# zju3dv/NeuralRecon-W

Hardware: AMD Instinct MI355X
Metric: ray-samples/sec (train step) at 1024 rays x 128 samples (higher is better)
Workload: dtype f16; 1 GPU; brandenburg_gate config (BASELINE.json configs[1]): 1024 rays/GPU x (64 coarse + 64 fine) samples, SDF 8x256 + colour 4x256 + bg NeRF 8x256, 4 outside samples, up_sample_steps 2, render+loss+backward+allreduce+clip+Adam; rays_per_gpu=1024, samples_per_ray=128, global_rays=1024, parallelism=dp1, world_size=1, submission=eager, streams=2, skipped_steps=0

## Files before the change

include/neuconw_hip.h:

```cpp
#ifndef NEUCONW_HIP_H
#define NEUCONW_HIP_H
#include <stdint.h>

#ifdef __cplusplus
extern "C" {
#endif

#define NCW_PREC_F32 0
#define NCW_PREC_BF16 1
#define NCW_PREC_F16 2
#define NCW_MAX_LAYERS 12
#define NCW_MAX_SEGS 4

#define NCW_E_BADARG (-1)
#define NCW_E_UNSUPPORTED (-2)

int ncw_abi_version(void);
const char* ncw_source_hash(void);
int ncw_device_info(char* buf, int buflen);

typedef struct NcwSeg {
    int32_t col0;
    int32_t ncols;
    int32_t dcol0;
// ... 136 lines not shown
    const void* w_p[8]; const void* wt_p[8]; const float* b_p[8];
    const void* w_alpha; const void* wt_alpha; const float* b_alpha;
    const void* w_feat; const void* wt_feat; const float* b_feat;
    const void* w_a[4]; const void* wt_a[4]; const float* b_a[4];
    const void* w_rgb; const void* wt_rgb; const float* b_rgb;
    int32_t D;
    int32_t skip;
    int32_t rbn, rbh, n_head, n_a;
    const void* w_p_lo[8]; const void* w_alpha_lo; const void* w_feat_lo; const void* w_a_lo[4]; const void* w_rgb_lo;
} NcwNerfNet;

typedef struct NcwNerfStash {
    void* gp;
    void* aux1;
    void* h[9];
    void* featn;
    void* e[4];
    void* zp[8];
    void* zalpha;
    void* zfeat;
    void* ze[4];
    void* zrgb;
    const float* aux_bias;
} NcwNerfStash;

int ncw_nerf_fwd(const NcwNerfNet* net, int prec, const NcwPoints* pts, const float* x4, int64_t n, const float* a,
                 float* density, float* rgb, const NcwNerfStash* stash, void* stream);
int ncw_nerf_bwd(const NcwNerfNet* net, int prec, const NcwPoints* pts, int64_t n, const float* d_density,
                 const float* d_rgb, float* d_a, float* d_a_rows, const NcwNerfStash* stash, void* stream);
int ncw_nerf_refine(const NcwNerfNet* net, int prec, const NcwPoints* pts, int64_t n, const float* aux_bias, float* density,
                    float* rgb, void* stream);
int ncw_batch_assemble(const float* all_rays, int ncols, const float* all_rgbs, const int64_t* idx, int64_t n_rows,
                       int64_t B, int with_semantics, float* rays, int64_t* ts, int64_t* label, float* rgbs,
                       const int* mask_ids, int n_ids, uint8_t* keep, void* stream);
int ncw_aux_ray_bias(const float* w, int ldw, int col0, int n_out, const float* rays_d, const float* a, int n_a, int64_t R,
                     float* out, int ldo, void* stream);
int ncw_ray_prologue(const float* rays, int ncols, int64_t R, const float* origin_host, float radius, float* rays_o,
                     float* rays_d, float* near, float* far, float* depth_gt, float* depth_weight, void* stream);
int ncw_inv_s_fwd(const float* variance, float* inv_s, float* s_val, void* stream);
int ncw_inv_s_bwd(const float* d_inv_s_rays, int64_t R, const float* inv_s, float* d_variance, void* stream);
int ncw_loss_fwd(const float* color, const float* rgbs, int64_t R, const float* gradient_error, const float* mask_error,
                 int64_t n_mask, const float* sfm, int64_t n_sfm, float coef, float igr_w, float mask_w, float depth_w,
                 float* loss, void* stream);
int ncw_loss_bwd(const float* d_loss, const float* color, const float* rgbs, int64_t R, int64_t n_mask, int64_t n_sfm,
                 float coef, float igr_w, float mask_w, float depth_w, float* d_color, float* d_gradient_error,
                 float* d_mask_error, float* d_sfm, void* stream);
// ... 325 lines not shown
```

neuralrecon-w_amd/csrc/ncw_mlp.h:

```cpp
#pragma once
#include "../../include/neuconw_hip.h"
#include "ncw_common.h"

template <class P>
struct Fast { static constexpr bool v = (P::id == NCW_PREC_BF16); };

NCW_DEV void ncw_lds_barrier() {
    asm volatile("s_waitcnt lgkmcnt(0)" ::: "memory");
    __builtin_amdgcn_s_barrier();
    asm volatile("" ::: "memory");
}

NCW_DEV float grid_linspace(float start, float end, int steps, int i) {
    if (steps == 1) return start;
    const float step = (end - start) / (float)(steps - 1);
    return (i < steps / 2) ? start + step * (float)i : end - step * (float)(steps - 1 - i);
}

NCW_DEV int64_t points_count(const NcwPoints& s, int64_t n) {
    if (s.mode != 4) return n;
    const int64_t c = (int64_t)s.count[0];
    return c < n ? c : n;
}
NCW_DEV int64_t point_slot(const NcwPoints& s, int64_t p) { return s.mode == 4 ? (int64_t)s.idx[p] : p; }
// ... 106 lines not shown
NCW_DEV void relu_epilogue(Act<P, RB>& act, CVec<RB>& acc, typename P::selem* st, size_t tile, int lane) {
#pragma unroll
    for (int rb = 0; rb < RB; ++rb) {
        f32x16 yv;
#pragma unroll
        for (int r = 0; r < 16; ++r) yv[r] = ncw_relu(acc.v[rb][r]);
        if (st) stash_store_block(st, tile, RB, rb, yv, lane);
        to_act_block<RB>(act, rb, yv);
    }
}

template <class P, int RB>
NCW_DEV void relu_backward(Act<P, RB>& za, const CVec<RB>& u, const typename P::selem* st_y, typename P::selem* st_z,
                           size_t tile, int lane) {
#pragma unroll
    for (int rb = 0; rb < RB; ++rb) {
        f32x16 y, z;
        stash_load_block(y, st_y, tile, RB, rb, lane);
#pragma unroll
        for (int r = 0; r < 16; ++r) z[r] = y[r] > 0.f ? u.v[rb][r] : 0.f;
        stash_store_block(st_z, tile, RB, rb, z, lane);
        to_act_block<RB>(za, rb, z);
    }
}

template <class P, int RB, int NX = 0>
struct SoftplusB {
    static constexpr int RB_IN = RB + NX;
    typedef typename P::selem SE;
    const CVec<RB>& z;
    SE* st_h;
    SE* st_s;
    size_t tile;
    int lane;
    const Act<P, (NX > 0 ? NX : 1)>* extra;
    Act<P, RB> act;
    NCW_DEV SoftplusB(const CVec<RB>& z_, SE* h, SE* s, size_t t, int l, const Act<P, (NX > 0 ? NX : 1)>* x = nullptr)
        : z(z_), st_h(h), st_s(s), tile(t), lane(l), extra(x) {}
    NCW_DEV void prepare(int rb) {
        if (rb >= RB) return;
        f32x16 yv, sv;
#pragma unroll
        for (int r = 0; r < 16; ++r) {
            float y, sg;
            softplus100<Fast<P>::v>(z.v[rb][r], y, sg);
            yv[r] = y;
// ... 173 lines not shown
```

neuralrecon-w_amd/csrc/ncw_sdf8.hip:

```cpp
#include "ncw_mlp.h"

namespace {

constexpr int SB_WAVES = 8, SB_TILES = 4;

NCW_DEV void load_sprime_block_bf16(f32x16& sv, const ncw_h16* __restrict__ st_h, size_t tile, int RB, int rb, int lane) {
    stash_load_block(sv, st_h, tile, RB, rb, lane);
#pragma unroll
    for (int r = 0; r < 16; ++r) sv[r] = 1.f - __builtin_amdgcn_exp2f(sv[r] * -144.26950408889634f);
}
constexpr int SB_ACT = SB_TILES * 16 * 1024;
constexpr int SB_GAM = SB_TILES * 3 * 1024;

typedef __attribute__((address_space(3))) bf16x8 sb_lfrag;

template <int NU>
NCW_DEV void sb_load_slice(bf16x8* a, const void* w, int rb_stride, int ob, int u0, int lane) {
#pragma unroll
    for (int q = 0; q < NU; ++q) a[q] = ncw_ld_frag<bf16x8>(w, (size_t)(u0 + q) * rb_stride + ob, lane);
}

constexpr int SB_RD = 4;

template <int NU, bool TWO, int NPF = 0>
// ... 230 lines not shown
        int comp;
        const float dv = freq_feature_deriv<3, 6, true>(xs, f0 + 4 * h, comp);
        const float c = gg[r] * dv;
        nx += comp == 0 ? c : 0.f;
        ny += comp == 1 ? c : 0.f;
        nz += comp == 2 ? c : 0.f;
    }
    nx = half_pair_sum(nx); ny = half_pair_sum(ny); nz = half_pair_sum(nz);
    typedef __attribute__((address_space(3))) float lfloat;
    lfloat* part = (lfloat*)gbuf;
    if (jb == 1 && lane < 32) {
        part[(jt * 32 + lane) * 3 + 0] = nx; part[(jt * 32 + lane) * 3 + 1] = ny; part[(jt * 32 + lane) * 3 + 2] = nz;
    }
    ncw_lds_barrier();
    if (jb == 0 && lane < 32 && valid) {
        grad[p * 3 + 0] = nx + part[(jt * 32 + lane) * 3 + 0];
        grad[p * 3 + 1] = ny + part[(jt * 32 + lane) * 3 + 1];
        grad[p * 3 + 2] = nz + part[(jt * 32 + lane) * 3 + 2];
    }
}


constexpr int SB_X = SB_TILES * 6 * 1024;

NCW_DEV void inverted_sphere8(const float (&x)[3], float (&p4)[4]) {
    float r2;
    {
#pragma clang fp contract(off)
        const float s1 = x[1] * x[1], s2 = x[2] * x[2];
        r2 = __builtin_fmaf(x[0], x[0], s1) + s2;
    }
    float r = sqrtf(r2);
    r = fminf(fmaxf(r, 1.0f), 1e10f);
    p4[0] = x[0] / r; p4[1] = x[1] / r; p4[2] = x[2] / r; p4[3] = 1.0f / r;
}

template <bool TRAIN>
__global__ __launch_bounds__(64 * SB_WAVES) void nerf_fwdB_kernel(NcwNerfNet net, NcwPoints src, const float* __restrict__ x4,
                                                                 int64_t n, const float* __restrict__ a,
                                                                 float* __restrict__ density, float* __restrict__ rgb,
                                                                 NcwNerfStash st) {
    typedef ncw_h16 SE;
    __shared__ __attribute__((aligned(16))) char lds[2 * SB_ACT + SB_X + SB_TILES * 32 * 4];
    sb_lfrag* const abuf0 = (sb_lfrag*)(ncw_lchar*)lds;
    sb_lfrag* const abuf1 = abuf0 + SB_ACT / 16;
    sb_lfrag* const xbuf = abuf0 + 2 * SB_ACT / 16;
    typedef __attribute__((address_space(3))) int sb_lint;
    sb_lint* const rbuf = (sb_lint*)(xbuf + SB_X / 16);
    const int lane = ncw_lane();
    const int wave = __builtin_amdgcn_readfirstlane((int)(threadIdx.x >> 6));
    const int64_t tile0 = (int64_t)blockIdx.x * SB_TILES;
    const int D = net.D;
    n = points_count(src, n);
    if (tile0 * 32 >= n) return;
    int64_t pp = 0;
    bool pvalid = false;
    if (wave < SB_TILES) {
        int64_t p = (tile0 + wave) * 32 + (lane & 31), ray;
        pvalid = p < n;
        if (!pvalid) p = n - 1;
// ... 28 lines not shown
        load_bias(b1, bp + ob * 32, lane);
        return b1.v[0];
    };
    auto relu16 = [](const f32x16& v) {
        f32x16 y;
#pragma unroll
        for (int r = 0; r < 16; ++r) y[r] = ncw_relu(v[r]);
        return y;
    };
    f32x16 bnext;
    {
        bf16x8 w0[6];
        const f32x16 bias = bias_of(net.b_p[0], wave);
        sb_load_slice<6>(w0, net.w_p[0], 8, wave, 0, lane);
        bnext = bias_of(D > 1 ? net.b_p[1] : net.b_feat, wave);
        sb_load_slice<16>(wa, D > 1 ? net.w_p[1] : net.w_feat, 8, wave, 0, lane);
        ncw_lds_barrier();
#pragma unroll
        for (int t = 0; t < SB_TILES; ++t) {
            f32x16 acc = bias;
            sb_mma<6, false>(acc, acc, w0, xbuf + t * 6 * 64 + lane, nullptr);
            const f32x16 y = relu16(acc);
            if (TRAIN) stash_store_block((SE*)st.h[1], (size_t)(tile0 + t), 8, wave, y, lane);
            sb_store_units(abuf0, t, wave, y, lane);
        }
    }
    int cur = 0;
    for (int i = 1; i < D; ++i) {
        const bool skip = (i == net.skip + 1);
        const void* wnext = i + 1 < D ? net.w_p[i + 1] : net.w_feat;
        const f32x16 bias = bnext;
        if (skip) sb_load_slice<6>(wx, net.w_p[i], 8, wave, 16, lane);
        bnext = bias_of(i + 1 < D ? net.b_p[i + 1] : net.b_feat, wave);
        ncw_lds_barrier();
        const sb_lfrag* in = cur ? abuf1 : abuf0;
        sb_lfrag* out = cur ? abuf0 : abuf1;
#pragma unroll
        for (int tp = 0; tp < SB_TILES; tp += 2) {
            f32x16 acc0 = bias, acc1 = bias;
            const sb_lfrag *in0 = in + tp * 16 * 64 + lane, *in1 = in0 + 16 * 64;
            if (tp == SB_TILES - 2) sb_mma<16, true, 16>(acc0, acc1, wa, in0, in1, wnext, 8, wave, lane);
            else sb_mma<16, true>(acc0, acc1, wa, in0, in1);
            if (skip) sb_mma<6, true>(acc0, acc1, wx, xbuf + tp * 6 * 64 + lane, xbuf + (tp + 1) * 6 * 64 + lane);
#pragma unroll
            for (int j = 0; j < 2; ++j) {
                const f32x16 y = relu16(j ? acc1 : acc0);
                if (TRAIN) stash_store_block((SE*)st.h[i + 1], (size_t)(tile0 + tp + j), 8, wave, y, lane);
                sb_store_units(out, tp + j, wave, y, lane);
            }
        }
        cur ^= 1;
    }
    const int hb = wave & 3, hp = wave >> 2;
    const int ta = 2 * hp, tb = 2 * hp + 1;
    {
        const f32x16 bias = bnext;
        ncw_lds_barrier();
        const sb_lfrag* in = cur ? abuf1 : abuf0;
        sb_lfrag* out = cur ? abuf0 : abuf1;
        if (wave < SB_TILES) {
            if (TRAIN || st.aux_bias == nullptr) {
                CVec<3> aux1;
                if (TRAIN) {
                    stash_load<3>(aux1, (const SE*)st.aux1, (size_t)(tile0 + wave), lane);
                } else {
                    const int64_t ray = rbuf[wave * 32 + (lane & 31)];
                    const float dir[3] = {src.rays_d[ray * 3 + 0], src.rays_d[ray * 3 + 1], src.rays_d[ray * 3 + 2]};
                    build_aux1<true>(aux1, dir, a + ray * net.n_a, net.n_a, lane);
                }
                Act<PrecBF16, 3> aux1a;
// ... 6 lines not shown
            sb_load_slice<16>(w1, net.w_alpha, 1, 0, 0, lane);
            CVec<1> o;
            load_bias(o, net.b_alpha, lane);
            sb_mma<16, false>(o.v[0], o.v[0], w1, in + wave * 16 * 64 + lane, nullptr);
            if (pvalid && lane < 32) density[pp] = o.v[0][0];
        }
        sb_load_slice<6>(wx, net.w_a[0], 4, hb, 16, lane);
        bnext = bias_of(net.b_a[0], hb);
#pragma unroll
        for (int tp = 0; tp < SB_TILES; tp += 2) {
            f32x16 acc0 = bias, acc1 = bias;
            const sb_lfrag *in0 = in + tp * 16 * 64 + lane, *in1 = in0 + 16 * 64;
            if (tp == SB_TILES - 2) sb_mma<16, true, 16>(acc0, acc1, wa, in0, in1, net.w_a[0], 4, hb, lane);
            else sb_mma<16, true>(acc0, acc1, wa, in0, in1);
            if (TRAIN) {
                stash_store_block((SE*)st.featn, (size_t)(tile0 + tp), 8, wave, acc0, lane);
                stash_store_block((SE*)st.featn, (size_t)(tile0 + tp + 1), 8, wave, acc1, lane);
            }
            sb_store_units(out, tp, wave, acc0, lane);
            sb_store_units(out, tp + 1, wave, acc1, lane);
        }
        cur ^= 1;
    }
    for (int i = 0; i < net.n_head; ++i) {
        const bool more = i + 1 < net.n_head;
        const f32x16 bias = bnext;
        if (more) bnext = bias_of(net.b_a[i + 1], hb);
        f32x16 rb0, rb1;
        const bool ray_rows = (i == 0 && st.aux_bias != nullptr);
        if (ray_rows) {
            auto ray_row = [&](int t) {
                const f32x4* ab = reinterpret_cast<const f32x4*>(st.aux_bias + (size_t)rbuf[t * 32 + (lane & 31)] * 128) + 8 * hb + (lane >> 5);
                f32x16 v;
#pragma unroll
                for (int g = 0; g < 4; ++g) {
                    const f32x4 q = ab[2 * g];
#pragma unroll
                    for (int c = 0; c < 4; ++c) v[4 * g + c] = q[c];
                }
                return v;
            };
            rb0 = ray_row(ta);
            rb1 = ray_row(tb);
        }
        ncw_lds_barrier();
        const sb_lfrag* in = cur ? abuf1 : abuf0;
        sb_lfrag* out = cur ? abuf0 : abuf1;
        const sb_lfrag *in0 = in + ta * 16 * 64 + lane, *in1 = in + tb * 16 * 64 + lane;
        const void* wnext = net.w_a[more ? i + 1 : i];
        f32x16 acc0 = bias, acc1 = bias;
        if (i == 0) {
            sb_mma<16, true, 8>(acc0, acc1, wa, in0, in1, wnext, 4, hb, lane);
            if (ray_rows) {
#pragma unroll
                for (int r = 0; r < 16; ++r) { acc0[r] += rb0[r]; acc1[r] += rb1[r]; }
            } else {
                sb_mma<6, true>(acc0, acc1, wx, xbuf + ta * 6 * 64 + lane, xbuf + tb * 6 * 64 + lane);
            }
        } else {
            sb_mma<8, true, 8>(acc0, acc1, wa, in0, in1, wnext, 4, hb, lane);
        }
        const f32x16 y0 = relu16(acc0), y1 = relu16(acc1);
        if (TRAIN) {
            stash_store_block((SE*)st.e[i], (size_t)(tile0 + ta), 4, hb, y0, lane);
            stash_store_block((SE*)st.e[i], (size_t)(tile0 + tb), 4, hb, y1, lane);
        }
        sb_store_units(out, ta, hb, y0, lane);
        sb_store_units(out, tb, hb, y1, lane);
        cur ^= 1;
    }
    ncw_lds_barrier();
    if (wave < SB_TILES) {
        const sb_lfrag* in = cur ? abuf1 : abuf0;
        bf16x8 w1[8];
        sb_load_slice<8>(w1, net.w_rgb, 1, 0, 0, lane);
        CVec<1> o;
        load_bias(o, net.b_rgb, lane);
        sb_mma<8, false>(o.v[0], o.v[0], w1, in + wave * 16 * 64 + lane, nullptr);
        if (pvalid && lane < 32) {
            rgb[pp * 3 + 0] = o.v[0][0];
            rgb[pp * 3 + 1] = o.v[0][1];
            rgb[pp * 3 + 2] = o.v[0][2];
        }
    }
}


typedef ncw_h16 sb_h4 __attribute__((ext_vector_type(4)));
struct SbMask { sb_h4 g[4]; };
NCW_DEV SbMask sb_mask_load(const ncw_h16* __restrict__ st_y, size_t tile, int RB, int rb, int lane) {
    const sb_h4* p = reinterpret_cast<const sb_h4*>(st_y) + ((tile * RB + rb) * 4) * 64 + lane;
    SbMask m;
#pragma unroll
    for (int g = 0; g < 4; ++g) m.g[g] = NCW_STASH_LD(p[g * 64]);
    return m;
}
NCW_DEV f32x16 sb_relu_bwd(const f32x16& u, const SbMask& m) {
    f32x16 z;
#pragma unroll
    for (int r = 0; r < 16; ++r) z[r] = (float)m.g[r >> 2][r & 3] > 0.f ? u[r] : 0.f;
    return z;
}

NCW_DEV void sb_accumulate_d_a(int rb, const f32x16& q, float* __restrict__ d_a, int64_t ray, int n_a, bool valid, int lane) {
    const int h = lane >> 5;
    const int64_t r0 = __shfl(ray, 0, 64);
    const bool uniform = __all((ray == r0) ? 1 : 0);
#pragma unroll
    for (int r = 0; r < 16; ++r) {
        const int f = 32 * rb + ncw_feat_of(r, 0) + 4 * h;
        const int j = f - 27;
        float v = valid ? q[r] : 0.f;
        if (uniform) {
#pragma unroll
            for (int o = 1; o < 32; o <<= 1) v += __shfl_xor(v, o, 64);
            if ((lane & 31) == 0 && j >= 0 && j < n_a) atomicAdd(d_a + ray * n_a + j, v);
        } else {
            if (valid && j >= 0 && j < n_a) atomicAdd(d_a + ray * n_a + j, v);
        }
    }
}

__global__ __launch_bounds__(64 * SB_WAVES) void nerf_bwdB_kernel(NcwNerfNet net, NcwPoints src, int64_t n,
                                                                 const float* __restrict__ d_density,
                                                                 const float* __restrict__ d_rgb, float* __restrict__ d_a,
                                                                 NcwNerfStash st) {
    typedef ncw_h16 SE;
    __shared__ __attribute__((aligned(16))) char lds[2 * SB_ACT + SB_X];
    sb_lfrag* const abuf0 = (sb_lfrag*)(ncw_lchar*)lds;
    sb_lfrag* const abuf1 = abuf0 + SB_ACT / 16;
    sb_lfrag* const xbuf = abuf0 + 2 * SB_ACT / 16;
    const int lane = ncw_lane();
    const int wave = __builtin_amdgcn_readfirstlane((int)(threadIdx.x >> 6));
    const int64_t tile0 = (int64_t)blockIdx.x * SB_TILES;
    const int D = net.D, NH = net.n_head;
    const int hb = wave & 3, hp = wave >> 2, ta = 2 * hp, tb = 2 * hp + 1;
    typedef const __attribute__((address_space(1))) bf16x8* gfrag;
    n = points_count(src, n);
    if (tile0 * 32 >= n) return;
    if (wave < SB_TILES) {
        int64_t p = (tile0 + wave) * 32 + (lane & 31);
        const bool valid = p < n;
        if (!valid) p = n - 1;
        p = point_slot(src, p);
        const float vm = valid ? 1.f : 0.f;
        CVec<1> zr, zal;
        cvec_zero(zr);
        cvec_zero(zal);
        if (lane < 32) {
            zr.v[0][0] = d_rgb[p * 3 + 0] * vm;
            zr.v[0][1] = d_rgb[p * 3 + 1] * vm;
            zr.v[0][2] = d_rgb[p * 3 + 2] * vm;
            zal.v[0][0] = d_density[p] * vm;
        }
        stash_store<1>((SE*)st.zrgb, (size_t)(tile0 + wave), zr, lane);
        stash_store<1>((SE*)st.zalpha, (size_t)(tile0 + wave), zal, lane);
        Act<PrecBF16, 1> za1;
        to_act(za1, zr);
        xbuf[(wave * 6 + 0) * 64 + lane] = za1.f[0];
        to_act(za1, zal);
        xbuf[(wave * 6 + 1) * 64 + lane] = za1.f[0];
    }
    bf16x8 wa[16];
    f32x16 zero16;
#pragma unroll
    for (int r = 0; r < 16; ++r) zero16[r] = 0.f;
    int cur = 0;
    SbMask m0, m1;
    f32x16 ue0, ue1;
    {
        const bf16x8 wr = ((gfrag)net.wt_rgb)[(size_t)hb * 64 + lane];
        m0 = sb_mask_load((const SE*)st.e[NH - 1], (size_t)(tile0 + ta), 4, hb, lane);
        m1 = sb_mask_load((const SE*)st.e[NH - 1], (size_t)(tile0 + tb), 4, hb, lane);
        if (NH > 1) sb_load_slice<8>(wa, net.wt_a[NH - 1], 4, hb, 0, lane);
        else sb_load_slice<8>(wa, net.wt_a[0], 11, wave, 0, lane);
        ncw_lds_barrier();
        ue0 = NCW_MFMA_H(wr, xbuf[(ta * 6 + 0) * 64 + lane], zero16, 0, 0, 0);
        ue1 = NCW_MFMA_H(wr, xbuf[(tb * 6 + 0) * 64 + lane], zero16, 0, 0, 0);
    }
    for (int i = NH - 1; i >= 1; --i) {
        sb_lfrag* out = cur ? abuf1 : abuf0;
        const f32x16 z0 = sb_relu_bwd(ue0, m0), z1 = sb_relu_bwd(ue1, m1);
        stash_store_block((SE*)st.ze[i], (size_t)(tile0 + ta), 4, hb, z0, lane);
        stash_store_block((SE*)st.ze[i], (size_t)(tile0 + tb), 4, hb, z1, lane);
        sb_store_units(out, ta, hb, z0, lane);
        sb_store_units(out, tb, hb, z1, lane);
        m0 = sb_mask_load((const SE*)st.e[i - 1], (size_t)(tile0 + ta), 4, hb, lane);
        m1 = sb_mask_load((const SE*)st.e[i - 1], (size_t)(tile0 + tb), 4, hb, lane);
        const bool head_next = i - 1 >= 1;
        const void* wnext = head_next ? net.wt_a[i - 1] : net.wt_a[0];
        const int sn = head_next ? 4 : 11, obn = head_next ? hb : wave;
        ncw_lds_barrier();
        ue0 = zero16; ue1 = zero16;
        sb_mma<8, true, 8>(ue0, ue1, wa, out + ta * 16 * 64 + lane, out + tb * 16 * 64 + lane, wnext, sn, obn, lane);
        cur ^= 1;
    }
    {
        sb_lfrag* out = cur ? abuf1 : abuf0;
        const f32x16 z0 = sb_relu_bwd(ue0, m0), z1 = sb_relu_bwd(ue1, m1);
        stash_store_block((SE*)st.ze[0], (size_t)(tile0 + ta), 4, hb, z0, lane);
        stash_store_block((SE*)st.ze[0], (size_t)(tile0 + tb), 4, hb, z1, lane);
        sb_store_units(out, ta, hb, z0, lane);
        sb_store_units(out, tb, hb, z1, lane);
        sb_load_slice<8>(wa + 8, net.wt_feat, 8, wave, 8, lane);
        bf16x8 wq[8];
        sb_load_slice<8>(wq, net.wt_a[0], 11, 8 + wave % 3, 0, lane);
        ncw_lds_barrier();
        const sb_lfrag* in = out;
        sb_lfrag* out2 = cur ? abuf0 : abuf1;
        for (int j = wave; j < 12; j += SB_WAVES) {
            const int b = j % 3, t = j / 3;
            if (j != wave) sb_load_slice<8>(wq, net.wt_a[0], 11, 8 + b, 0, lane);
            int64_t p = (tile0 + t) * 32 + (lane & 31);
            const bool valid = p < n;
            if (!valid) p = n - 1;
            p = point_slot(src, p);
            const int64_t ray = (src.mode == 0) ? p : p / src.per_ray;
            f32x16 qa = zero16;
            sb_mma<8, false>(qa, qa, wq, in + t * 16 * 64 + lane, nullptr);
            sb_accumulate_d_a(b, qa, d_a, ray, net.n_a, valid, lane);
        }
#pragma unroll
        for (int tp = 0; tp < SB_TILES; tp += 2) {
            f32x16 a0 = zero16, a1 = zero16;
            const sb_lfrag *in0 = in + tp * 16 * 64 + lane, *in1 = in0 + 16 * 64;
            if (tp == SB_TILES - 2) sb_mma<8, true, 8>(a0, a1, wa, in0, in1, net.wt_feat, 8, wave, lane);
            else sb_mma<8, true>(a0, a1, wa, in0, in1);
            stash_store_block((SE*)st.zfeat, (size_t)(tile0 + tp), 8, wave, a0, lane);
            stash_store_block((SE*)st.zfeat, (size_t)(tile0 + tp + 1), 8, wave, a1, lane);
            sb_store_units(out2, tp, wave, a0, lane);
            sb_store_units(out2, tp + 1, wave, a1, lane);
        }
        cur ^= 1;
    }
    auto sweep = [&](const SE* st_h, SE* st_z, const bf16x8* wal, const void* wnext, int sn, bool store) __attribute__((always_inline)) {
        ncw_lds_barrier();
        const sb_lfrag* in = cur ? abuf1 : abuf0;
        sb_lfrag* out = cur ? abuf0 : abuf1;
#pragma unroll
        for (int tp = 0; tp < SB_TILES; tp += 2) {
            m0 = sb_mask_load(st_h, (size_t)(tile0 + tp), 8, wave, lane);
            m1 = sb_mask_load(st_h, (size_t)(tile0 + tp + 1), 8, wave, lane);
            f32x16 u0 = zero16, u1 = zero16;
            const sb_lfrag *in0 = in + tp * 16 * 64 + lane, *in1 = in0 + 16 * 64;
            if (tp == SB_TILES - 2) sb_mma<16, true, 16>(u0, u1, wa, in0, in1, wnext, sn, wave, lane);
            else sb_mma<16, true>(u0, u1, wa, in0, in1);
            if (wal != nullptr) {
                u0 = NCW_MFMA_H(*wal, xbuf[(tp * 6 + 1) * 64 + lane], u0, 0, 0, 0);
                u1 = NCW_MFMA_H(*wal, xbuf[((tp + 1) * 6 + 1) * 64 + lane], u1, 0, 0, 0);
            }
            const f32x16 z0 = sb_relu_bwd(u0, m0), z1 = sb_relu_bwd(u1, m1);
            stash_store_block(st_z, (size_t)(tile0 + tp), 8, wave, z0, lane);
            stash_store_block(st_z, (size_t)(tile0 + tp + 1), 8, wave, z1, lane);
            if (store) {
                sb_store_units(out, tp, wave, z0, lane);
                sb_store_units(out, tp + 1, wave, z1, lane);
            }
        }
        cur ^= 1;
    };
    {
        const bf16x8 wal = ((gfrag)net.wt_alpha)[(size_t)wave * 64 + lane];
        sweep((const SE*)st.h[D], (SE*)st.zp[D - 1], &wal, net.wt_p[D - 1], (D - 1 == net.skip + 1) ? 11 : 8, true);
    }
    for (int i = D - 1; i >= 1; --i) {
        const int ln = i - 1 >= 1 ? i - 1 : i;
        sweep((const SE*)st.h[i], (SE*)st.zp[i - 1], nullptr, net.wt_p[ln], (ln == net.skip + 1) ? 11 : 8, i - 1 >= 1);
    }
}


}

int NCW_FN(ncw_sdf_fwd8_launch)(const NcwSdfNet* net, const NcwPoints& src, int64_t n, float* sdf, float* grad, const NcwSdfStash& stash,
                        hipStream_t st) {
    const int64_t tiles = (n + 31) / 32;
    if (stash.t[0] == nullptr)
        hipLaunchKernelGGL(sdf_fwdB_kernel<false>, dim3((unsigned)((tiles + SB_TILES - 1) / SB_TILES)), dim3(64 * SB_WAVES), 0, st,
                           *net, src, n, sdf, grad, stash);
    else
        hipLaunchKernelGGL(sdf_fwdB_kernel<true>, dim3((unsigned)((tiles + SB_TILES - 1) / SB_TILES)), dim3(64 * SB_WAVES), 0, st,
                           *net, src, n, sdf, grad, stash);
    NCW_CHECK_LAUNCH();
    return 0;
}

int NCW_FN(ncw_nerf_fwd8_launch)(const NcwNerfNet* net, const NcwPoints& src, const float* x4, int64_t n, const float* a, float* density,
                         float* rgb, const NcwNerfStash& stash, hipStream_t st) {
    const int64_t tiles = (n + 31) / 32;
    if (stash.gp == nullptr)
        hipLaunchKernelGGL(nerf_fwdB_kernel<false>, dim3((unsigned)((tiles + SB_TILES - 1) / SB_TILES)), dim3(64 * SB_WAVES), 0, st,
                           *net, src, x4, n, a, density, rgb, stash);
    else
        hipLaunchKernelGGL(nerf_fwdB_kernel<true>, dim3((unsigned)((tiles + SB_TILES - 1) / SB_TILES)), dim3(64 * SB_WAVES), 0, st,
                           *net, src, x4, n, a, density, rgb, stash);
    NCW_CHECK_LAUNCH();
    return 0;
}

int NCW_FN(ncw_nerf_bwd8_launch)(const NcwNerfNet* net, const NcwPoints& src, int64_t n, const float* d_density, const float* d_rgb,
                         float* d_a, const NcwNerfStash& stash, hipStream_t st) {
    const int64_t tiles = (n + 31) / 32;
    hipLaunchKernelGGL(nerf_bwdB_kernel, dim3((unsigned)((tiles + SB_TILES - 1) / SB_TILES)), dim3(64 * SB_WAVES), 0, st, *net, src, n,
                       d_density, d_rgb, d_a, stash);
    NCW_CHECK_LAUNCH();
    return 0;
}
```

neuralrecon-w_amd/lib.py:

```python
import ctypes as C
import os

HERE = os.path.dirname(os.path.abspath(__file__))
LIB_PATH = os.environ.get("NEUCONW_HIP_LIB") or os.path.join(HERE, "libneuconw_hip.so")

PREC_F32 = 0
PREC_BF16 = 1
PREC_F16 = 2
MAX_LAYERS = 12
MAX_SEGS = 4
ABI_VERSION = 32


class NcwSeg(C.Structure):
    _fields_ = [("col0", C.c_int32), ("ncols", C.c_int32), ("dcol0", C.c_int32), ("_pad", C.c_int32)]


class NcwPackDesc(C.Structure):
    _fields_ = [
        ("src", C.c_void_p), ("g", C.c_void_p), ("bias", C.c_void_p), ("dst_w", C.c_void_p), ("dst_b", C.c_void_p),
        ("ld", C.c_int32), ("row0", C.c_int32), ("nrows", C.c_int32), ("drow0", C.c_int32),
        ("rb_out", C.c_int32), ("rb_in", C.c_int32), ("transpose", C.c_int32), ("prec", C.c_int32),
        ("scale", C.c_float), ("nseg", C.c_int32), ("seg", NcwSeg * MAX_SEGS), ("residual", C.c_int32), ("_pad", C.c_int32),
    ]
# ... 102 lines not shown


class NcwColorStash(C.Structure):
    _fields_ = [("aux1", C.c_void_p), ("aux2", C.c_void_p), ("f", C.c_void_p), ("e", C.c_void_p * 4),
                ("x", C.c_void_p * 8), ("zf", C.c_void_p), ("ze", C.c_void_p * 4), ("zx", C.c_void_p * 8),
                ("zo", C.c_void_p), ("aux_bias", C.c_void_p)]


class NcwNerfNet(C.Structure):
    _fields_ = [("w_p", C.c_void_p * 8), ("wt_p", C.c_void_p * 8), ("b_p", C.c_void_p * 8),
                ("w_alpha", C.c_void_p), ("wt_alpha", C.c_void_p), ("b_alpha", C.c_void_p),
                ("w_feat", C.c_void_p), ("wt_feat", C.c_void_p), ("b_feat", C.c_void_p),
                ("w_a", C.c_void_p * 4), ("wt_a", C.c_void_p * 4), ("b_a", C.c_void_p * 4),
                ("w_rgb", C.c_void_p), ("wt_rgb", C.c_void_p), ("b_rgb", C.c_void_p),
                ("D", C.c_int32), ("skip", C.c_int32), ("rbn", C.c_int32), ("rbh", C.c_int32),
                ("n_head", C.c_int32), ("n_a", C.c_int32),
                ("w_p_lo", C.c_void_p * 8), ("w_alpha_lo", C.c_void_p), ("w_feat_lo", C.c_void_p), ("w_a_lo", C.c_void_p * 4),
                ("w_rgb_lo", C.c_void_p)]


class NcwNerfStash(C.Structure):
    _fields_ = [("gp", C.c_void_p), ("aux1", C.c_void_p), ("h", C.c_void_p * 9), ("featn", C.c_void_p),
                ("e", C.c_void_p * 4), ("zp", C.c_void_p * 8), ("zalpha", C.c_void_p), ("zfeat", C.c_void_p),
                ("ze", C.c_void_p * 4), ("zrgb", C.c_void_p), ("aux_bias", C.c_void_p)]


def _ptr_struct(name, fields_ptr, fields_other=()):
    return type(name, (C.Structure,), {"_fields_": [(f, C.c_void_p) for f in fields_ptr] + list(fields_other)})


NcwCompositeIn = _ptr_struct(
    "NcwCompositeIn",
    ["rays_o", "rays_d", "z", "z_feed", "sample_dist", "sdf", "grad", "rgb", "density", "bg_rgb", "inv_s",
     "background_rgb", "cos_anneal_dev"],
    [("cos_anneal", C.c_float), ("R", C.c_int32), ("S", C.c_int32), ("O", C.c_int32), ("has_bg", C.c_int32),
     ("trim_sphere", C.c_int32)],
)
NcwCompositeOut = _ptr_struct(
    "NcwCompositeOut",
    ["color", "color_sphere", "color_bg", "weights", "weights_sum", "cdf", "inside", "depth", "normals", "eik",
     "mid_z", "dists", "bg_alpha", "weights_max"],
)
NcwCompositeGrad = _ptr_struct(
    "NcwCompositeGrad",
    ["d_color", "d_weights_sum", "d_depth", "d_eik_num", "d_sdf", "d_grad", "d_rgb", "d_density", "d_bg_rgb",
     "d_inv_s"],
    [("grad_scale", C.c_float), ("grad_scale_dev", C.c_void_p), ("d_normals", C.c_void_p)],
# ... 213 lines not shown
```

neuralrecon-w_amd/nerf.py:

```python
import ctypes
import os
from collections import OrderedDict

import torch
from torch import nn

from . import lib as L
from .neuconw import default_prec, points_struct, ray_head_bias
from .packing import PackPlan, _PackedNet
from .stash import StashCache, build_stash


class NeRF(_PackedNet):

    def __init__(self, D=8, W=256, d_in=3, d_in_view=3, multires=0, multires_view=0, output_ch=4, skips=[4],
                 in_channels_a=48, in_channels_dir=27, encode_appearance=False, use_viewdirs=False):
        super().__init__()
        if not (use_viewdirs and encode_appearance and d_in == 4 and d_in_view == 3 and multires == 10
                and multires_view == 4):
            raise NotImplementedError("HIP NeRF kernels implement the background configuration of "
                                      "lightning_modules/neuconw_system.py:90-103 only")
        if W not in (64, 256) or D < 2 or D > 8 or len(skips) != 1 or not (0 <= skips[0] < D - 1) or in_channels_a > 69:
            raise NotImplementedError("W in {64,256}, 2<=D<=8, one skip, n_a<=69")
        self.D, self.W, self.skips = D, W, list(skips)
        self.in_channels_a, self.in_channels_dir = in_channels_a, in_channels_dir
        self.input_ch, self.input_ch_view = 4 + 4 * 2 * multires, 3 + 3 * 2 * multires_view
        self.encode_appearance, self.use_viewdirs = encode_appearance, use_viewdirs
        self.pts_linears = nn.ModuleList(
            [nn.Linear(self.input_ch, W)]
            + [nn.Linear(W, W) if i not in self.skips else nn.Linear(W + self.input_ch, W) for i in range(D - 1)])
        od = OrderedDict([("static_linear_0", nn.Linear(W + in_channels_dir + in_channels_a, W // 2))])
        for i in range(1, D // 2):
            od["static_linear_%d" % i] = nn.Linear(W // 2, W // 2)
# ... 29 lines not shown
                sl["p%d" % i] = plan.add_linear(self.pts_linears[i], RBN, RBN, [(0, W, 0)], lo=split)
        sl["alpha"] = plan.add_linear(self.alpha_linear, 1, RBN, [(0, W, 0)], lo=split)
        sl["feat"] = plan.add_linear(self.feature_linear, RBN, RBN, [(0, W, 0)], lo=split)
        sl["a0"] = plan.add_linear(self.apperence_encoding[0], RBH, RBN + 3, [(0, W, 0), (W, 27 + A, 32 * RBN)], lo=split)
        for i in range(1, self.n_head):
            sl["a%d" % i] = plan.add_linear(self.apperence_encoding[i], RBH, RBH, [(0, W // 2, 0)], lo=split)
        sl["rgb"] = plan.add_linear(self.rgb_linear, 1, RBH, [(0, W // 2, 0)], lo=split)
        plan.finalize()
        for i in range(self.D):
            net.w_p[i], net.b_p[i], net.wt_p[i] = plan.wb_ptrs(sl["p%d" % i])
            net.w_p_lo[i] = plan.mat_ptr(sl["p%d" % i].lo)
        for i in range(self.n_head):
            net.w_a[i], net.b_a[i], net.wt_a[i] = plan.wb_ptrs(sl["a%d" % i])
            net.w_a_lo[i] = plan.mat_ptr(sl["a%d" % i].lo)
        net.w_alpha, net.b_alpha, net.wt_alpha = plan.wb_ptrs(sl["alpha"])
        net.w_feat, net.b_feat, net.wt_feat = plan.wb_ptrs(sl["feat"])
        net.w_rgb, net.b_rgb, net.wt_rgb = plan.wb_ptrs(sl["rgb"])
        net.w_alpha_lo, net.w_feat_lo, net.w_rgb_lo = (plan.mat_ptr(sl[k].lo) for k in ("alpha", "feat", "rgb"))
        plan.has_lo = split
        net.D, net.skip, net.rbn, net.rbh, net.n_head, net.n_a = self.D, self.skips[0], RBN, RBH, self.n_head, A
        plan.net, plan.slots = net, sl
        return plan

    def _stash_fields(self, train):
        RBN, RBH = self.W // 32, self.W // 64
        if not train:
            return []
        return [("gp", 3), ("aux1", 3), ("featn", RBN), ("zalpha", 1), ("zfeat", RBN), ("zrgb", 1),
                ("h", {i: RBN for i in range(1, self.D + 1)}), ("zp", [RBN] * self.D), ("e", [RBH] * self.n_head),
                ("ze", [RBH] * self.n_head)]

    def fwd_stash(self, pts, n, prec, a, x4=None, select=None, train=True, refine=None):
        dev = self._first_param().device
        plan = self.packed(prec)
        ent = self.__dict__.setdefault("_stash_cache", StashCache()).acquire(
            (prec, n, str(dev), bool(train)), lambda: build_stash(L.NcwNerfStash, self._stash_fields(train), dev, prec, n))
        ar, ids, st = ent["arena"], ent["ids"], ent["stash"]
        sel_count = None
        do_refine = (refine is not None and prec == L.PREC_F16 and self.refine and getattr(plan, "has_lo", False) and x4 is None)
        pts_sel = None
        if select is not None or do_refine:
            z_prim, O_ = select if select is not None else refine
            z_prim = z_prim.contiguous().float()
            S_ = int(z_prim.shape[1])
            assert x4 is None and pts.mode == 2 and pts.per_ray == S_ + O_
            if "sel_idx" not in ent:
                ent["sel_idx"] = torch.empty(n, device=dev, dtype=torch.int32)
                ent["sel_count"] = torch.zeros(1, device=dev, dtype=torch.int32)
                ent["sel_offs"] = torch.empty(n // (S_ + O_) + 1, device=dev, dtype=torch.int32)
            sel_count = ent["sel_count"]
            L.check(L.get_lib().ncw_bg_select(pts.rays_o, pts.rays_d, L.ptr(z_prim), pts.sample_dist, n // (S_ + O_), S_, O_,
                                              L.ptr(ent["sel_idx"]), L.ptr(ent["sel_offs"]), L.ptr(sel_count),
                                              L.stream_ptr(dev)), "ncw_bg_select")
            if train and select is not None:
                from .stash import SelectionProbe

                probe = self.__dict__.get("_sel_probe")
                if probe is None and not torch.cuda.is_current_stream_capturing():
                    probe = self._sel_probe = SelectionProbe()
# ... 72 lines not shown
```

neuralrecon-w_amd/stash.py:

```python

import os
from typing import NamedTuple

import torch

from . import lib as L


class StashArena:

    def __init__(self, device, prec, n_points):
        self.device = torch.device(device)
        self.prec = prec
        self.n = int(n_points)
        self.tiles = (self.n + 31) // 32
        self.tiles_alloc = (self.tiles + 23) // 24 * 24
        self.esize = 4 if prec == L.PREC_F32 else 2
        self._off = []
        self._bytes = 0
        self.buf = None

    def new(self, rb):
        off = self._bytes
        self._bytes += self.tiles_alloc * rb * 1024 * self.esize
        self._bytes = (self._bytes + 255) & ~255
        self._off.append((off, rb))
        return len(self._off) - 1

    def allocate(self, zero=False):
        fn = torch.zeros if zero else torch.empty
        self.buf = fn(max(self._bytes, 256), dtype=torch.uint8, device=self.device)
        return self

    def ptr(self, i):
        return self.buf.data_ptr() + self._off[i][0]

    def rb(self, i):
        return self._off[i][1]

    def to_rows(self, i, F):
        out = torch.empty(self.n, F, device=self.device, dtype=torch.float32)
        L.check(L.get_lib().ncw_stash_to_rows(self.prec, self.ptr(i), self.n, F, self.rb(i), L.ptr(out),
                                              L.stream_ptr(self.device)), "ncw_stash_to_rows")
        return out

    def from_rows(self, i, rows):
        rows = rows.contiguous().float()
        assert rows.shape[0] == self.n
        L.check(L.get_lib().ncw_stash_from_rows(self.prec, L.ptr(rows), self.n, rows.shape[1], self.rb(i),
                                                self.ptr(i), L.stream_ptr(self.device)), "ncw_stash_from_rows")


def build_stash(struct_type, fields, device, prec, n_points):
    ar = StashArena(device, prec, n_points)
    ids = {}
    for name, rb in fields:
        if isinstance(rb, dict):
            ids[name] = {l: ar.new(r) for l, r in rb.items()}
        else:
            ids[name] = [ar.new(r) for r in rb] if isinstance(rb, list) else ar.new(rb)
    ar.allocate()
    st = struct_type()
    for name, i in ids.items():
        if isinstance(i, int):
            setattr(st, name, ar.ptr(i))
        else:
            for l, v in (i.items() if isinstance(i, dict) else enumerate(i)):
                getattr(st, name)[l] = ar.ptr(v)
    return dict(arena=ar, ids=ids, stash=st)


class WgradProduct(NamedTuple):
    x: int
    rbx: int
    y: int
    rby: int
    dense: int
    ld: int
    dbias: int
    n: int
    n_dev: int
    frac: float

# ... 174 lines not shown
```

Before: 33.05 million ray-samples/s.

## Store 1-bit ReLU masks for bg NeRF backward instead of reloading fp16 activations

The background NeRF forward kernel now also writes packed 1-bit ReLU masks per 16-element block for the trunk and head layers. The backward kernel reads these masks instead of reloading the full 16-bit activation stash to gate gradients. This cuts backward read traffic per layer by about 16x, at the cost of extra mask computation and stores in the forward pass. The full activation stash is still written, so forward writes grow a little and total memory use increases.

```diff
diff --git a/include/neuconw_hip.h b/include/neuconw_hip.h
--- a/include/neuconw_hip.h
+++ b/include/neuconw_hip.h
@@ -182,6 +182,8 @@
     void* ze[4];
     void* zrgb;
     const float* aux_bias;
+    void* hm[9];
+    void* em[4];
 } NcwNerfStash;
 
 int ncw_nerf_fwd(const NcwNerfNet* net, int prec, const NcwPoints* pts, const float* x4, int64_t n, const float* a,
diff --git a/neuralrecon-w_amd/csrc/ncw_mlp.h b/neuralrecon-w_amd/csrc/ncw_mlp.h
--- a/neuralrecon-w_amd/csrc/ncw_mlp.h
+++ b/neuralrecon-w_amd/csrc/ncw_mlp.h
@@ -152,6 +152,45 @@
         stash_store_block(st_z, tile, RB, rb, z, lane);
         to_act_block<RB>(za, rb, z);
     }
+}
+
+typedef unsigned short ncw_mask16;
+NCW_HD constexpr int ncw_mask_bit(int r) { return (r >> 1) + 8 * (r & 1); }
+template <class SE>
+NCW_DEV uint32_t relu_mask_bits(const f32x16& y) {
+    typedef unsigned short u16x2 __attribute__((ext_vector_type(2)));
+    static_assert(__is_same(SE, _Float16) || __is_same(SE, __bf16), "1-bit ReLU masks: 16-bit stash elements only");
+    constexpr unsigned short INF = __is_same(SE, _Float16) ? 0x7C00 : 0x7F80;
+    uint32_t m = 0;
+#pragma unroll
+    for (int k = 0; k < 8; ++k) {
+        u16x2 h;
+        h[0] = __builtin_bit_cast(unsigned short, (SE)y[2 * k]);
+        h[1] = __builtin_bit_cast(unsigned short, (SE)y[2 * k + 1]);
+        u16x2 t = h - (unsigned short)1;
+        t = __builtin_elementwise_min(t, (u16x2)INF);
+        t = ((u16x2)INF - t + (unsigned short)0x7FFF) >> 15;
+        m |= __builtin_bit_cast(uint32_t, t) << k;
+    }
+    return (m | (m >> 8)) & 0xFFFFu;
+}
+NCW_DEV void mask_store_block(void* __restrict__ base, size_t tile, int RB, int rb, uint32_t bits, int lane) {
+    char* blk = reinterpret_cast<char*>(base) + (tile * RB + rb) * 128;
+    NCW_STASH_ST(*reinterpret_cast<ncw_mask16*>(blk + (uint32_t)lane * 2u), (ncw_mask16)bits);
+}
+NCW_DEV uint32_t mask_load_block(const void* __restrict__ base, size_t tile, int RB, int rb, int lane) {
+    const char* blk = reinterpret_cast<const char*>(base) + (tile * RB + rb) * 128;
+    return NCW_STASH_LD(*reinterpret_cast<const ncw_mask16*>(blk + (uint32_t)lane * 2u));
+}
+NCW_DEV f32x16 mask_apply_block(const f32x16& u, uint32_t bits) {
+    f32x16 z;
+#pragma unroll
+    for (int r = 0; r < 16; ++r) {
+        const int keep = (int)(bits << (31 - ncw_mask_bit(r))) >> 31;
+        const float ur = u[r];
+        z[r] = __builtin_bit_cast(float, __builtin_bit_cast(int, ur) & keep);
+    }
+    return z;
 }
 
 template <class P, int RB, int NX = 0>
diff --git a/neuralrecon-w_amd/csrc/ncw_sdf8.hip b/neuralrecon-w_amd/csrc/ncw_sdf8.hip
--- a/neuralrecon-w_amd/csrc/ncw_sdf8.hip
+++ b/neuralrecon-w_amd/csrc/ncw_sdf8.hip
@@ -276,6 +276,8 @@
 
 
 constexpr int SB_X = SB_TILES * 6 * 1024;
+template <bool V>
+struct SbConst { static constexpr bool value = V; };
 
 NCW_DEV void inverted_sphere8(const float (&x)[3], float (&p4)[4]) {
     float r2;
@@ -289,7 +291,7 @@
     p4[0] = x[0] / r; p4[1] = x[1] / r; p4[2] = x[2] / r; p4[3] = 1.0f / r;
 }
 
-template <bool TRAIN>
+template <bool TRAIN, bool BITS>
 __global__ __launch_bounds__(64 * SB_WAVES) void nerf_fwdB_kernel(NcwNerfNet net, NcwPoints src, const float* __restrict__ x4,
                                                                  int64_t n, const float* __restrict__ a,
                                                                  float* __restrict__ density, float* __restrict__ rgb,
@@ -364,6 +366,7 @@
             sb_mma<6, false>(acc, acc, w0, xbuf + t * 6 * 64 + lane, nullptr);
             const f32x16 y = relu16(acc);
             if (TRAIN) stash_store_block((SE*)st.h[1], (size_t)(tile0 + t), 8, wave, y, lane);
+            if (BITS) mask_store_block(st.hm[1], (size_t)(tile0 + t), 8, wave, relu_mask_bits<SE>(y), lane);
             sb_store_units(abuf0, t, wave, y, lane);
         }
     }
@@ -388,6 +391,7 @@
             for (int j = 0; j < 2; ++j) {
                 const f32x16 y = relu16(j ? acc1 : acc0);
                 if (TRAIN) stash_store_block((SE*)st.h[i + 1], (size_t)(tile0 + tp + j), 8, wave, y, lane);
+                if (BITS) mask_store_block(st.hm[i + 1], (size_t)(tile0 + tp + j), 8, wave, relu_mask_bits<SE>(y), lane);
                 sb_store_units(out, tp + j, wave, y, lane);
             }
         }
@@ -440,12 +444,13 @@
         }
         cur ^= 1;
     }
-    for (int i = 0; i < net.n_head; ++i) {
+    auto head_layer = [&](int i, auto first) __attribute__((always_inline)) {
+        constexpr bool FIRST = decltype(first)::value;
         const bool more = i + 1 < net.n_head;
         const f32x16 bias = bnext;
         if (more) bnext = bias_of(net.b_a[i + 1], hb);
         f32x16 rb0, rb1;
-        const bool ray_rows = (i == 0 && st.aux_bias != nullptr);
+        const bool ray_rows = (FIRST && st.aux_bias != nullptr);
         if (ray_rows) {
             auto ray_row = [&](int t) {
                 const f32x4* ab = reinterpret_cast<const f32x4*>(st.aux_bias + (size_t)rbuf[t * 32 + (lane & 31)] * 128) + 8 * hb + (lane >> 5);
@@ -467,7 +472,7 @@
         const sb_lfrag *in0 = in + ta * 16 * 64 + lane, *in1 = in + tb * 16 * 64 + lane;
         const void* wnext = net.w_a[more ? i + 1 : i];
         f32x16 acc0 = bias, acc1 = bias;
-        if (i == 0) {
+        if constexpr (FIRST) {
             sb_mma<16, true, 8>(acc0, acc1, wa, in0, in1, wnext, 4, hb, lane);
             if (ray_rows) {
 #pragma unroll
@@ -483,10 +488,16 @@
             stash_store_block((SE*)st.e[i], (size_t)(tile0 + ta), 4, hb, y0, lane);
             stash_store_block((SE*)st.e[i], (size_t)(tile0 + tb), 4, hb, y1, lane);
         }
+        if (BITS) {
+            mask_store_block(st.em[i], (size_t)(tile0 + ta), 4, hb, relu_mask_bits<SE>(y0), lane);
+            mask_store_block(st.em[i], (size_t)(tile0 + tb), 4, hb, relu_mask_bits<SE>(y1), lane);
+        }
         sb_store_units(out, ta, hb, y0, lane);
         sb_store_units(out, tb, hb, y1, lane);
         cur ^= 1;
-    }
+    };
+    head_layer(0, SbConst<true>{});
+    for (int i = 1; i < net.n_head; ++i) head_layer(i, SbConst<false>{});
     ncw_lds_barrier();
     if (wave < SB_TILES) {
         const sb_lfrag* in = cur ? abuf1 : abuf0;
@@ -505,19 +516,34 @@
 
 
 typedef ncw_h16 sb_h4 __attribute__((ext_vector_type(4)));
+template <bool BITS>
 struct SbMask { sb_h4 g[4]; };
-NCW_DEV SbMask sb_mask_load(const ncw_h16* __restrict__ st_y, size_t tile, int RB, int rb, int lane) {
-    const sb_h4* p = reinterpret_cast<const sb_h4*>(st_y) + ((tile * RB + rb) * 4) * 64 + lane;
-    SbMask m;
-#pragma unroll
-    for (int g = 0; g < 4; ++g) m.g[g] = NCW_STASH_LD(p[g * 64]);
+template <>
+struct SbMask<true> { uint32_t bits; };
+template <bool BITS>
+NCW_DEV SbMask<BITS> sb_mask_load(const void* __restrict__ st_y, const void* __restrict__ st_m, size_t tile, int RB, int rb, int lane) {
+    SbMask<BITS> m;
+    if constexpr (BITS) {
+        m.bits = mask_load_block(st_m, tile, RB, rb, lane);
+    } else {
+        const sb_h4* p = reinterpret_cast<const sb_h4*>(st_y) + ((tile * RB + rb) * 4) * 64 + lane;
+#pragma unroll
+        for (int g = 0; g < 4; ++g) m.g[g] = NCW_STASH_LD(p[g * 64]);
+    }
     return m;
 }
-NCW_DEV f32x16 sb_relu_bwd(const f32x16& u, const SbMask& m) {
-    f32x16 z;
-#pragma unroll
-    for (int r = 0; r < 16; ++r) z[r] = (float)m.g[r >> 2][r & 3] > 0.f ? u[r] : 0.f;
-    return z;
+template <bool BITS>
+NCW_DEV f32x16 sb_relu_bwd(const f32x16& u, const SbMask<BITS>& m) {
+    if constexpr (BITS) {
+        uint32_t bits = m.bits;
+        asm volatile("" : "+v"(bits));
+        return mask_apply_block(u, bits);
+    } else {
+        f32x16 z;
+#pragma unroll
+        for (int r = 0; r < 16; ++r) z[r] = (float)m.g[r >> 2][r & 3] > 0.f ? u[r] : 0.f;
+        return z;
+    }
 }
 
 NCW_DEV void sb_accumulate_d_a(int rb, const f32x16& q, float* __restrict__ d_a, int64_t ray, int n_a, bool valid, int lane) {
@@ -539,6 +565,7 @@
     }
 }
 
+template <bool BITS>
 __global__ __launch_bounds__(64 * SB_WAVES) void nerf_bwdB_kernel(NcwNerfNet net, NcwPoints src, int64_t n,
                                                                  const float* __restrict__ d_density,
                                                                  const float* __restrict__ d_rgb, float* __restrict__ d_a,
@@ -584,12 +611,12 @@
 #pragma unroll
     for (int r = 0; r < 16; ++r) zero16[r] = 0.f;
     int cur = 0;
-    SbMask m0, m1;
+    SbMask<BITS> m0, m1;
     f32x16 ue0, ue1;
     {
         const bf16x8 wr = ((gfrag)net.wt_rgb)[(size_t)hb * 64 + lane];
-        m0 = sb_mask_load((const SE*)st.e[NH - 1], (size_t)(tile0 + ta), 4, hb, lane);
-        m1 = sb_mask_load((const SE*)st.e[NH - 1], (size_t)(tile0 + tb), 4, hb, lane);
+        m0 = sb_mask_load<BITS>(st.e[NH - 1], st.em[NH - 1], (size_t)(tile0 + ta), 4, hb, lane);
+        m1 = sb_mask_load<BITS>(st.e[NH - 1], st.em[NH - 1], (size_t)(tile0 + tb), 4, hb, lane);
         if (NH > 1) sb_load_slice<8>(wa, net.wt_a[NH - 1], 4, hb, 0, lane);
         else sb_load_slice<8>(wa, net.wt_a[0], 11, wave, 0, lane);
         ncw_lds_barrier();
@@ -603,8 +630,8 @@
         stash_store_block((SE*)st.ze[i], (size_t)(tile0 + tb), 4, hb, z1, lane);
         sb_store_units(out, ta, hb, z0, lane);
         sb_store_units(out, tb, hb, z1, lane);
-        m0 = sb_mask_load((const SE*)st.e[i - 1], (size_t)(tile0 + ta), 4, hb, lane);
-        m1 = sb_mask_load((const SE*)st.e[i - 1], (size_t)(tile0 + tb), 4, hb, lane);
+        m0 = sb_mask_load<BITS>(st.e[i - 1], st.em[i - 1], (size_t)(tile0 + ta), 4, hb, lane);
+        m1 = sb_mask_load<BITS>(st.e[i - 1], st.em[i - 1], (size_t)(tile0 + tb), 4, hb, lane);
         const bool head_next = i - 1 >= 1;
         const void* wnext = head_next ? net.wt_a[i - 1] : net.wt_a[0];
         const int sn = head_next ? 4 : 11, obn = head_next ? hb : wave;
@@ -651,14 +678,14 @@
         }
         cur ^= 1;
     }
-    auto sweep = [&](const SE* st_h, SE* st_z, const bf16x8* wal, const void* wnext, int sn, bool store) __attribute__((always_inline)) {
+    auto sweep = [&](const void* st_h, const void* st_m, SE* st_z, const bf16x8* wal, const void* wnext, int sn, bool store) __attribute__((always_inline)) {
         ncw_lds_barrier();
         const sb_lfrag* in = cur ? abuf1 : abuf0;
         sb_lfrag* out = cur ? abuf0 : abuf1;
 #pragma unroll
         for (int tp = 0; tp < SB_TILES; tp += 2) {
-            m0 = sb_mask_load(st_h, (size_t)(tile0 + tp), 8, wave, lane);
-            m1 = sb_mask_load(st_h, (size_t)(tile0 + tp + 1), 8, wave, lane);
+            m0 = sb_mask_load<BITS>(st_h, st_m, (size_t)(tile0 + tp), 8, wave, lane);
+            m1 = sb_mask_load<BITS>(st_h, st_m, (size_t)(tile0 + tp + 1), 8, wave, lane);
             f32x16 u0 = zero16, u1 = zero16;
             const sb_lfrag *in0 = in + tp * 16 * 64 + lane, *in1 = in0 + 16 * 64;
             if (tp == SB_TILES - 2) sb_mma<16, true, 16>(u0, u1, wa, in0, in1, wnext, sn, wave, lane);
@@ -667,8 +694,9 @@
                 u0 = NCW_MFMA_H(*wal, xbuf[(tp * 6 + 1) * 64 + lane], u0, 0, 0, 0);
                 u1 = NCW_MFMA_H(*wal, xbuf[((tp + 1) * 6 + 1) * 64 + lane], u1, 0, 0, 0);
             }
-            const f32x16 z0 = sb_relu_bwd(u0, m0), z1 = sb_relu_bwd(u1, m1);
+            const f32x16 z0 = sb_relu_bwd(u0, m0);
             stash_store_block(st_z, (size_t)(tile0 + tp), 8, wave, z0, lane);
+            const f32x16 z1 = sb_relu_bwd(u1, m1);
             stash_store_block(st_z, (size_t)(tile0 + tp + 1), 8, wave, z1, lane);
             if (store) {
                 sb_store_units(out, tp, wave, z0, lane);
@@ -679,11 +707,11 @@
     };
     {
         const bf16x8 wal = ((gfrag)net.wt_alpha)[(size_t)wave * 64 + lane];
-        sweep((const SE*)st.h[D], (SE*)st.zp[D - 1], &wal, net.wt_p[D - 1], (D - 1 == net.skip + 1) ? 11 : 8, true);
+        sweep(st.h[D], st.hm[D], (SE*)st.zp[D - 1], &wal, net.wt_p[D - 1], (D - 1 == net.skip + 1) ? 11 : 8, true);
     }
     for (int i = D - 1; i >= 1; --i) {
         const int ln = i - 1 >= 1 ? i - 1 : i;
-        sweep((const SE*)st.h[i], (SE*)st.zp[i - 1], nullptr, net.wt_p[ln], (ln == net.skip + 1) ? 11 : 8, i - 1 >= 1);
+        sweep(st.h[i], st.hm[i], (SE*)st.zp[i - 1], nullptr, net.wt_p[ln], (ln == net.skip + 1) ? 11 : 8, i - 1 >= 1);
     }
 }
 
@@ -706,12 +734,13 @@
 int NCW_FN(ncw_nerf_fwd8_launch)(const NcwNerfNet* net, const NcwPoints& src, const float* x4, int64_t n, const float* a, float* density,
                          float* rgb, const NcwNerfStash& stash, hipStream_t st) {
     const int64_t tiles = (n + 31) / 32;
+    const dim3 grid((unsigned)((tiles + SB_TILES - 1) / SB_TILES)), block(64 * SB_WAVES);
     if (stash.gp == nullptr)
-        hipLaunchKernelGGL(nerf_fwdB_kernel<false>, dim3((unsigned)((tiles + SB_TILES - 1) / SB_TILES)), dim3(64 * SB_WAVES), 0, st,
-                           *net, src, x4, n, a, density, rgb, stash);
+        hipLaunchKernelGGL((nerf_fwdB_kernel<false, false>), grid, block, 0, st, *net, src, x4, n, a, density, rgb, stash);
+    else if (stash.hm[1] == nullptr)
+        hipLaunchKernelGGL((nerf_fwdB_kernel<true, false>), grid, block, 0, st, *net, src, x4, n, a, density, rgb, stash);
     else
-        hipLaunchKernelGGL(nerf_fwdB_kernel<true>, dim3((unsigned)((tiles + SB_TILES - 1) / SB_TILES)), dim3(64 * SB_WAVES), 0, st,
-                           *net, src, x4, n, a, density, rgb, stash);
+        hipLaunchKernelGGL((nerf_fwdB_kernel<true, true>), grid, block, 0, st, *net, src, x4, n, a, density, rgb, stash);
     NCW_CHECK_LAUNCH();
     return 0;
 }
@@ -719,8 +748,11 @@
 int NCW_FN(ncw_nerf_bwd8_launch)(const NcwNerfNet* net, const NcwPoints& src, int64_t n, const float* d_density, const float* d_rgb,
                          float* d_a, const NcwNerfStash& stash, hipStream_t st) {
     const int64_t tiles = (n + 31) / 32;
-    hipLaunchKernelGGL(nerf_bwdB_kernel, dim3((unsigned)((tiles + SB_TILES - 1) / SB_TILES)), dim3(64 * SB_WAVES), 0, st, *net, src, n,
-                       d_density, d_rgb, d_a, stash);
+    const dim3 grid((unsigned)((tiles + SB_TILES - 1) / SB_TILES)), block(64 * SB_WAVES);
+    if (stash.hm[1] == nullptr)
+        hipLaunchKernelGGL(nerf_bwdB_kernel<false>, grid, block, 0, st, *net, src, n, d_density, d_rgb, d_a, stash);
+    else
+        hipLaunchKernelGGL(nerf_bwdB_kernel<true>, grid, block, 0, st, *net, src, n, d_density, d_rgb, d_a, stash);
     NCW_CHECK_LAUNCH();
     return 0;
 }
diff --git a/neuralrecon-w_amd/lib.py b/neuralrecon-w_amd/lib.py
--- a/neuralrecon-w_amd/lib.py
+++ b/neuralrecon-w_amd/lib.py
@@ -148,7 +148,8 @@
 class NcwNerfStash(C.Structure):
     _fields_ = [("gp", C.c_void_p), ("aux1", C.c_void_p), ("h", C.c_void_p * 9), ("featn", C.c_void_p),
                 ("e", C.c_void_p * 4), ("zp", C.c_void_p * 8), ("zalpha", C.c_void_p), ("zfeat", C.c_void_p),
-                ("ze", C.c_void_p * 4), ("zrgb", C.c_void_p), ("aux_bias", C.c_void_p)]
+                ("ze", C.c_void_p * 4), ("zrgb", C.c_void_p), ("aux_bias", C.c_void_p),
+                ("hm", C.c_void_p * 9), ("em", C.c_void_p * 4)]
 
 
 def _ptr_struct(name, fields_ptr, fields_other=()):
diff --git a/neuralrecon-w_amd/nerf.py b/neuralrecon-w_amd/nerf.py
--- a/neuralrecon-w_amd/nerf.py
+++ b/neuralrecon-w_amd/nerf.py
@@ -8,7 +8,7 @@
 from . import lib as L
 from .neuconw import default_prec, points_struct, ray_head_bias
 from .packing import PackPlan, _PackedNet
-from .stash import StashCache, build_stash
+from .stash import MaskBits, StashCache, build_stash
 
 
 class NeRF(_PackedNet):
@@ -84,19 +84,22 @@
         plan.net, plan.slots = net, sl
         return plan
 
-    def _stash_fields(self, train):
+    def _stash_fields(self, train, prec=None):
         RBN, RBH = self.W // 32, self.W // 64
         if not train:
             return []
-        return [("gp", 3), ("aux1", 3), ("featn", RBN), ("zalpha", 1), ("zfeat", RBN), ("zrgb", 1),
-                ("h", {i: RBN for i in range(1, self.D + 1)}), ("zp", [RBN] * self.D), ("e", [RBH] * self.n_head),
-                ("ze", [RBH] * self.n_head)]
+        fields = [("gp", 3), ("aux1", 3), ("featn", RBN), ("zalpha", 1), ("zfeat", RBN), ("zrgb", 1),
+                  ("h", {i: RBN for i in range(1, self.D + 1)}), ("zp", [RBN] * self.D), ("e", [RBH] * self.n_head),
+                  ("ze", [RBH] * self.n_head)]
+        if prec in (L.PREC_BF16, L.PREC_F16) and self.W == 256:
+            fields += [("hm", MaskBits({i: RBN for i in range(1, self.D + 1)})), ("em", MaskBits([RBH] * self.n_head))]
+        return fields
 
     def fwd_stash(self, pts, n, prec, a, x4=None, select=None, train=True, refine=None):
         dev = self._first_param().device
         plan = self.packed(prec)
         ent = self.__dict__.setdefault("_stash_cache", StashCache()).acquire(
-            (prec, n, str(dev), bool(train)), lambda: build_stash(L.NcwNerfStash, self._stash_fields(train), dev, prec, n))
+            (prec, n, str(dev), bool(train)), lambda: build_stash(L.NcwNerfStash, self._stash_fields(train, prec), dev, prec, n))
         ar, ids, st = ent["arena"], ent["ids"], ent["stash"]
         sel_count = None
         do_refine = (refine is not None and prec == L.PREC_F16 and self.refine and getattr(plan, "has_lo", False) and x4 is None)
diff --git a/neuralrecon-w_amd/stash.py b/neuralrecon-w_amd/stash.py
--- a/neuralrecon-w_amd/stash.py
+++ b/neuralrecon-w_amd/stash.py
@@ -8,6 +8,8 @@
 
 
 class StashArena:
+
+    MASK_BLOCK_BYTES = 128
 
     def __init__(self, device, prec, n_points):
         self.device = torch.device(device)
@@ -17,6 +19,7 @@
         self.tiles_alloc = (self.tiles + 23) // 24 * 24
         self.esize = 4 if prec == L.PREC_F32 else 2
         self._off = []
+        self._masks = set()
         self._bytes = 0
         self.buf = None
 
@@ -27,6 +30,34 @@
         self._off.append((off, rb))
         return len(self._off) - 1
 
+    def new_mask(self, rb):
+        off = self._bytes
+        self._bytes += self.tiles_alloc * rb * self.MASK_BLOCK_BYTES
+        self._bytes = (self._bytes + 255) & ~255
+        self._off.append((off, rb))
+        self._masks.add(len(self._off) - 1)
+        return len(self._off) - 1
+
+    def is_mask(self, i):
+        return i in self._masks
+
+    def nbytes(self, i):
+        return self.tiles_alloc * self.rb(i) * (self.MASK_BLOCK_BYTES if i in self._masks else 1024 * self.esize)
+
+    def mask_rows(self, i):
+        assert i in self._masks
+        rb = self.rb(i)
+        off = self._off[i][0]
+        w = self.buf[off:off + self.tiles * rb * self.MASK_BLOCK_BYTES].view(torch.int16).to(torch.int32) & 0xFFFF
+        w = w.view(self.tiles, rb, 2, 32)
+        r = torch.arange(16, device=self.device)
+        bits = ((w.unsqueeze(-1) >> ((r >> 1) + 8 * (r & 1))) & 1).bool()
+        feat = (r & 3) + 8 * (r >> 2)
+        out = torch.zeros(self.tiles, 32, rb, 32, dtype=torch.bool, device=self.device)
+        for h in (0, 1):
+            out[:, :, :, feat + 4 * h] = bits[:, :, h].permute(0, 2, 1, 3)
+        return out.reshape(self.tiles * 32, rb * 32)[:self.n]
+
     def allocate(self, zero=False):
         fn = torch.zeros if zero else torch.empty
         self.buf = fn(max(self._bytes, 256), dtype=torch.uint8, device=self.device)
@@ -51,14 +82,23 @@
                                                 self.ptr(i), L.stream_ptr(self.device)), "ncw_stash_from_rows")
 
 
+class MaskBits:
+
+    def __init__(self, spec):
+        self.spec = spec
+
+
 def build_stash(struct_type, fields, device, prec, n_points):
     ar = StashArena(device, prec, n_points)
     ids = {}
     for name, rb in fields:
+        new = ar.new
+        if isinstance(rb, MaskBits):
+            new, rb = ar.new_mask, rb.spec
         if isinstance(rb, dict):
-            ids[name] = {l: ar.new(r) for l, r in rb.items()}
+            ids[name] = {l: new(r) for l, r in rb.items()}
         else:
-            ids[name] = [ar.new(r) for r in rb] if isinstance(rb, list) else ar.new(rb)
+            ids[name] = [new(r) for r in rb] if isinstance(rb, list) else new(rb)
     ar.allocate()
     st = struct_type()
     for name, i in ids.items():
```

Measured after the change: 32.93 million ray-samples/s. No clear change (-0.4%).
